# hyye/lio-mapping

Hardware: AMD Instinct MI355X
Metric: sliding-window solves/sec, 64-line 130k-pt scans, window=15 (opt_window=5) (higher is better)
Workload: dtype f64 (solve) / f32 (features); 1 GPU; HDL-64E outdoor_test_config_64, S_outdoor ray-cast scans, window_size=15 opt_window_size=5, one SolveOptimization per step, clouds resident in HBM; n_lidar_residuals=78236, local_map_points=76752, surf_stack_points=19386, parallelism=1 window

## Files before the change

### lio-mapping_amd/csrc/cloud_device.h

```cpp
#pragma once
#include <hip/hip_runtime.h>

#include <cfloat>
#include <climits>
#include <cstddef>

#include "cloud_kernels.h"
#include "hmath.h"
#include "knn_merge.h"

#if defined(__HIPCC__)
namespace lio {

__device__ inline bool finite3(const float4 &p) { return isfinite(p.x) && isfinite(p.y) && isfinite(p.z); }
__device__ inline bool finite3(const Vec3<float> &p) { return isfinite(p.x) && isfinite(p.y) && isfinite(p.z); }


template <bool NORMALISE_CONJ>
__device__ __forceinline__ float4 to_end_point(float4 p, float s, const Quat<float> &qe, const Vec3<float> &te) {
  p.x -= s * te.x; p.y -= s * te.y; p.z -= s * te.z;
  Quat<float> qid;
  Quat<float> qs = slerp(qid, s, qe, FLT_EPSILON);
  Quat<float> qc = conj(qs);
  if (NORMALISE_CONJ) qc = normalized(qc);
  Vec3<float> v = rotate(qc, Vec3<float>(p.x, p.y, p.z));
  v = rotate(qe, v);
  p.x = v.x + te.x; p.y = v.y + te.y; p.z = v.z + te.z;
  return p;
}
template <bool KEEP>
__device__ __forceinline__ float4 deskew_to_end_point(float4 p, const Quat<float> &qe, const Vec3<float> &te, float time_factor) {
  float s = time_factor * (p.w - int(p.w));
  if (!KEEP) p.w -= int(p.w);
  return to_end_point<true>(p, s, qe, te);
}
__device__ __forceinline__ float4 affine_map_point(const float *__restrict__ m, const float4 &p) {
  float4 o;
  o.x = m[0] * p.x + m[1] * p.y + m[2] * p.z + m[3];
  o.y = m[4] * p.x + m[5] * p.y + m[6] * p.z + m[7];
  o.z = m[8] * p.x + m[9] * p.y + m[10] * p.z + m[11];
  o.w = p.w;
  return o;
}
template <class B> __device__ __forceinline__ const float4 *concat_src(B *base, const float4 *p) { return rebase(base, p); }
__device__ __forceinline__ const float4 *concat_src(std::nullptr_t, const float4 *p) { return p; }
template <class B>
__device__ __forceinline__ float4 concat_point(const ConcatSeg *__restrict__ seg, int nseg, int g, B base) {
  int sidx = 0;
  for (int k = 1; k < nseg; ++k)
    if (g >= seg[k].dst_off) sidx = k;
  const ConcatSeg &sg = seg[sidx];
  const float4 p = concat_src(base, sg.src)[g - sg.dst_off];
  float4 o;
  if (sg.identity) o = p;
  else o = affine_map_point(sg.tf.m, p);
  if (sg.set_intensity) o.w = sg.intensity;
  return o;
}
__device__ __forceinline__ void odo_to_end_body(const float4 *in, float4 *out, const int i, const OdomState *__restrict__ st, float time_factor,
                                                int no_deskew) {
  Quat<float> qe(st->T[3], st->T[0], st->T[1], st->T[2]);
  Vec3<float> te(st->T[4], st->T[5], st->T[6]);
  float4 p = in[i];
  float s = time_factor * (p.w - int(p.w));
  if (no_deskew) s = 0;
  p.w = float(int(p.w));
  out[i] = to_end_point<false>(p, s, qe, te);
}
__device__ __forceinline__ float4 rigid_map_point(float4 p, const Quat<float> &q, const Vec3<float> &t) {
  const Vec3<float> v = rotate(q, Vec3<float>(p.x, p.y, p.z));
  return make_float4(v.x + t.x, v.y + t.y, v.z + t.z, p.w);
}

__device__ inline int cell_coord(float v, float inv_cell) { return int(floorf(v * inv_cell)); }
__device__ __forceinline__ bool cell_of(float x, float y, float z, const GridDesc &g, int &cx, int &cy, int &cz) {
  cx = cell_coord(x, g.inv_cell) - g.origin[0];
  cy = cell_coord(y, g.inv_cell) - g.origin[1];
  cz = cell_coord(z, g.inv_cell) - g.origin[2];
  return cx >= 0 && cy >= 0 && cz >= 0 && cx < g.dims[0] && cy < g.dims[1] && cz < g.dims[2];
}
__device__ __forceinline__ uint32_t cell_index(int cx, int cy, int cz, const GridDesc &g) { return uint32_t(cx + g.dims[0] * (cy + g.dims[1] * cz)); }
__device__ __forceinline__ uint32_t cell_key_clamped(const float4 &p, const GridDesc &g) {
  int cx, cy, cz;
  cell_of(p.x, p.y, p.z, g, cx, cy, cz);
  cx = min(max(cx, 0), g.dims[0] - 1); cy = min(max(cy, 0), g.dims[1] - 1); cz = min(max(cz, 0), g.dims[2] - 1);
  return cell_index(cx, cy, cz, g);
}

__device__ __forceinline__ void cell_count_point(const float4 *__restrict__ pts, int i, const GridDesc &g, uint32_t *__restrict__ keys,
                                                 uint32_t *__restrict__ slot, int *__restrict__ cnt) {
  const uint32_t c = cell_key_clamped(pts[i], g);
  keys[i] = c;
  slot[i] = uint32_t(atomicAdd(&cnt[c], 1));
}
__device__ __forceinline__ void cell_place_point(const float4 *__restrict__ pts, const uint32_t *__restrict__ keys, const uint32_t *__restrict__ slot, int i,
                                                 const int *__restrict__ starts, float4 *__restrict__ sorted, int *__restrict__ cnt) {
  float4 p = pts[i];
  p.w = __int_as_float(i);
  const uint32_t c = keys[i];
  sorted[starts[c] + int(slot[i])] = p;
  cnt[c] = 0;
}

#define SEG_SCAN_THREADS 1024
#define SEG_SCAN_ITEMS 4
__device__ __forceinline__ void block_exclusive_scan(const int *__restrict__ in, int *__restrict__ out, int n, int base) {
  __shared__ int wsum[SEG_SCAN_THREADS / 64];
  const int tid = threadIdx.x, lane = tid & 63, wv = tid >> 6;
  int carry = base;
  for (int c0 = 0; c0 < n; c0 += SEG_SCAN_THREADS * SEG_SCAN_ITEMS) {
    const int i0 = c0 + tid * SEG_SCAN_ITEMS;
    int v[SEG_SCAN_ITEMS], tsum = 0;
#pragma unroll
    for (int k = 0; k < SEG_SCAN_ITEMS; ++k) { v[k] = i0 + k < n ? in[i0 + k] : 0; tsum += v[k]; }
    int inc = tsum;
#pragma unroll
    for (int off = 1; off < 64; off <<= 1) {
      const int u = __shfl_up(inc, off, 64);
      if (lane >= off) inc += u;
    }
    if (lane == 63) wsum[wv] = inc;
    __syncthreads();
    int before = 0, total = 0;
#pragma unroll
    for (int w = 0; w < SEG_SCAN_THREADS / 64; ++w) { const int t = wsum[w]; if (w < wv) before += t; total += t; }
    int run = carry + before + inc - tsum;
#pragma unroll
    for (int k = 0; k < SEG_SCAN_ITEMS; ++k)
      if (i0 + k < n) { out[i0 + k] = run; run += v[k]; }
    carry += total;
    __syncthreads();
  }
}

#define VOX_TILE 256
#define VOX_KEY_NONE 0xFFFFFFFFu

template <int ZBITS>
__device__ __forceinline__ bool vox_abs_key(const float4 &p, float inv_leaf, uint32_t &key) {
  constexpr int ZOFF = 1 << (ZBITS - 1);
  const float cx = floorf(p.x * inv_leaf), cy = floorf(p.y * inv_leaf), cz = floorf(p.z * inv_leaf);
  if (!(fabsf(cx) < 1024.f && fabsf(cy) < 1024.f && fabsf(cz) < float(ZOFF - 1))) return false;
  key = (uint32_t(int(cz) + ZOFF) << 22) | (uint32_t(int(cy) + 1024) << 11) | uint32_t(int(cx) + 1024);
  return true;
}
template <int ZBITS, uint32_t NONE>
__device__ __forceinline__ uint32_t vox_take_point(const float4 &p, float inv_leaf, float (&mn)[3], float (&mx)[3], float &cnt, int *__restrict__ flag) {
  uint32_t key = NONE;
  if (finite3(p)) {
    cnt = 1.f;
    mn[0] = mx[0] = p.x; mn[1] = mx[1] = p.y; mn[2] = mx[2] = p.z;
    if (!vox_abs_key<ZBITS>(p, inv_leaf, key)) *flag = 1;
  }
  return key;
}

__device__ __forceinline__ void vox_block_partial(float (&mn)[3], float (&mx)[3], float cnt, float *__restrict__ row) {
  __shared__ float sm[7][VOX_TILE / 64];
  const int lane = threadIdx.x & 63, wv = threadIdx.x >> 6;
#pragma unroll
  for (int o = 32; o > 0; o >>= 1) {
    for (int d = 0; d < 3; ++d) { mn[d] = fminf(mn[d], __shfl_xor(mn[d], o, 64)); mx[d] = fmaxf(mx[d], __shfl_xor(mx[d], o, 64)); }
    cnt += __shfl_xor(cnt, o, 64);
  }
  if (lane == 0) { for (int d = 0; d < 3; ++d) { sm[d][wv] = mn[d]; sm[3 + d][wv] = mx[d]; } sm[6][wv] = cnt; }
  __syncthreads();
  if (threadIdx.x < 7) {
    const int t = threadIdx.x;
    float v = sm[t][0];
    for (int w = 1; w < VOX_TILE / 64; ++w) v = t < 3 ? fminf(v, sm[t][w]) : (t < 6 ? fmaxf(v, sm[t][w]) : v + sm[t][w]);
    row[t] = v;
  }
}
__device__ __forceinline__ void cloud_bounds_block(const float4 *__restrict__ pts, int n, int block, int nb, float *__restrict__ row) {
  float mn[3] = {FLT_MAX, FLT_MAX, FLT_MAX}, mx[3] = {-FLT_MAX, -FLT_MAX, -FLT_MAX};
  float cnt = 0;
  for (int i = block * VOX_TILE + threadIdx.x; i < n; i += nb * VOX_TILE) {
    const float4 p = pts[i];
    if (!finite3(p)) continue;
    cnt += 1.f;
    mn[0] = fminf(mn[0], p.x); mn[1] = fminf(mn[1], p.y); mn[2] = fminf(mn[2], p.z);
    mx[0] = fmaxf(mx[0], p.x); mx[1] = fmaxf(mx[1], p.y); mx[2] = fmaxf(mx[2], p.z);
  }
  vox_block_partial(mn, mx, cnt, row);
}

__device__ __forceinline__ bool vox_fold_bounds(const float *__restrict__ partial, int nb, float inv_leaf, VoxParams &v) {
  __shared__ float sm[7][VOX_TILE];
  const int t = threadIdx.x;
  float mn[3] = {FLT_MAX, FLT_MAX, FLT_MAX}, mx[3] = {-FLT_MAX, -FLT_MAX, -FLT_MAX};
  float cnt = 0;
  for (int b = t; b < nb; b += VOX_TILE) {
    for (int d = 0; d < 3; ++d) { mn[d] = fminf(mn[d], partial[size_t(b) * 8 + d]); mx[d] = fmaxf(mx[d], partial[size_t(b) * 8 + 3 + d]); }
    cnt += partial[size_t(b) * 8 + 6];
  }
  for (int d = 0; d < 3; ++d) { sm[d][t] = mn[d]; sm[3 + d][t] = mx[d]; }
  sm[6][t] = cnt;
  __syncthreads();
  for (int st = VOX_TILE / 2; st > 0; st >>= 1) {
    if (t < st) {
      for (int d = 0; d < 3; ++d) { sm[d][t] = fminf(sm[d][t], sm[d][t + st]); sm[3 + d][t] = fmaxf(sm[3 + d][t], sm[3 + d][t + st]); }
      sm[6][t] += sm[6][t + st];
    }
    __syncthreads();
  }
  if (t != 0) return false;
  long long dd[3];
  for (int d = 0; d < 3; ++d) {
    v.mn[d] = sm[d][0]; v.mx[d] = sm[3 + d][0];
    dd[d] = (long long)((v.mx[d] - v.mn[d]) * inv_leaf) + 1;
    v.minb[d] = int(floorf(v.mn[d] * inv_leaf));
    const int maxb = int(floorf(v.mx[d] * inv_leaf));
    v.divb[d] = maxb - v.minb[d] + 1;
  }
  v.overflow = (sm[6][0] > 0 && dd[0] * dd[1] * dd[2] > (long long)INT_MAX) ? 1 : 0;
  v.n_valid = int(sm[6][0]);
  return true;
}

__device__ __forceinline__ bool vox_is_head(const uint32_t *__restrict__ keys, int i, uint32_t k) {
  return k != VOX_KEY_NONE && (i == 0 || keys[i - 1] != k);
}
__device__ __forceinline__ void vox_tile_head_count(const uint32_t *__restrict__ keys, int n, int tile, int *__restrict__ count) {
  __shared__ int swave[VOX_TILE / 64];
  const int i = tile * VOX_TILE + threadIdx.x;
  const uint32_t k = i < n ? keys[i] : VOX_KEY_NONE;
  const unsigned long long b = __ballot(vox_is_head(keys, i, k));
  if ((threadIdx.x & 63) == 0) swave[threadIdx.x >> 6] = __popcll(b);
  __syncthreads();
  if (threadIdx.x == 0) *count = (swave[0] + swave[1]) + (swave[2] + swave[3]);
}

struct VoxSlot { int pos; bool head; };
__device__ __forceinline__ VoxSlot vox_centroid_tile(const float4 *__restrict__ pts, const uint32_t *__restrict__ keys, const uint32_t *__restrict__ vals,
                                                     const int *__restrict__ tile_heads, int n, int tile, float4 *__restrict__ out) {
  __shared__ float4 sp[VOX_TILE];
  __shared__ uint32_t sk[VOX_TILE];
  __shared__ int swave[VOX_TILE / 64], sbase[VOX_TILE / 64];
  const int tid = threadIdx.x, lane = tid & 63, wv = tid >> 6;
  const int base_i = tile * VOX_TILE, i = base_i + tid;
  int before = 0;
  for (int b = tid; b < tile; b += VOX_TILE) before += tile_heads[b];
#pragma unroll
  for (int o = 32; o > 0; o >>= 1) before += __shfl_xor(before, o, 64);
  const uint32_t k = i < n ? keys[i] : VOX_KEY_NONE;
  sk[tid] = k;
  if (k != VOX_KEY_NONE) sp[tid] = pts[vals[i]];
  const bool head = vox_is_head(keys, i, k);
  const unsigned long long hb = __ballot(head);
  if (lane == 0) { swave[wv] = __popcll(hb); sbase[wv] = before; }
  __syncthreads();
  int pos = (sbase[0] + sbase[1]) + (sbase[2] + sbase[3]);
  for (int w = 0; w < wv; ++w) pos += swave[w];
  pos += __popcll(hb & ((1ull << lane) - 1ull));
  if (head) {
    float ax = 0, ay = 0, az = 0, ai = 0;
    int e = tid;
    while (e < VOX_TILE && sk[e] == k) { const float4 p = sp[e]; ax += p.x; ay += p.y; az += p.z; ai += p.w; ++e; }
    int cnt = e - tid;
    if (e == VOX_TILE) {
      int g = base_i + VOX_TILE;
      while (g < n && keys[g] == k) { const float4 p = pts[vals[g]]; ax += p.x; ay += p.y; az += p.z; ai += p.w; ++g; ++cnt; }
    }
    const float c = float(cnt);
    out[pos] = make_float4(ax / c, ay / c, az / c, ai / c);
  }
  return VoxSlot{pos, head};
}

#define VSORT_THREADS 256
#define VSORT_SCATTER_THREADS 512
#define VSORT_SCATTER_ITEMS 2

__device__ __forceinline__ unsigned long long vsort_from_lane(unsigned long long v, int byte_addr) {
  const uint32_t lo = uint32_t(__builtin_amdgcn_ds_bpermute(byte_addr, int(uint32_t(v))));
  const uint32_t hi = uint32_t(__builtin_amdgcn_ds_bpermute(byte_addr, int(uint32_t(v >> 32))));
  return (static_cast<unsigned long long>(hi) << 32) | lo;
}

template <int E>
__device__ __forceinline__ void vsort_block(unsigned long long (&v)[E], unsigned long long *__restrict__ lds) {
  constexpr int P = VSORT_THREADS * E;
  const int base = int(threadIdx.x) * E, lane = int(threadIdx.x) & 63;
#pragma unroll 1
  for (int k = 2; k <= P; k <<= 1) {
// ... 599 lines not shown
```

### lio-mapping_amd/csrc/cloud_kernels.h

```cpp
#pragma once
#include <algorithm>
#include <cmath>
#include <cstdint>

#include "dev.h"
#include "hmath.h"

namespace lio {

struct VoxParams {
  float mn[3], mx[3];
  int minb[3], divb[3];
  int overflow;
  int n_valid;
};

struct Affine3f { float m[12]; };

#define LIO_MAX_FRAMES 32

struct ConcatSeg { const float4 *src; int n; int dst_off; int identity; int set_intensity; float intensity; Affine3f tf; };
struct ConcatArgs { ConcatSeg seg[LIO_MAX_FRAMES]; int nseg; int total; };
void launch_transform_concat(const ConcatArgs &a, float4 *dst, hipStream_t s);

void launch_deskew_to_end(float4 *pts, int n, const float q[4], const float p[3], float time_factor, hipStream_t s, bool keep_intensity = false);
void launch_rigid_map(const float4 *in, int n, const float q[4], const float p[3], float4 *out, hipStream_t s);

inline int cloud_bounds_blocks(int n) { return std::max(1, std::min(cdiv(n, 256), 512)); }
struct BoundsSeg { const float4 *pts; int n, nb, off; };
void launch_seg_bounds(const BoundsSeg *d_segs, int nseg, int max_nb, float *partial, float inv_leaf, VoxParams *d_out, hipStream_t s);

#define VSORT_CAP 4096
#define VSORT_MEAN 384
#define VSORT_OVERSAMPLE 8
#define VSORT_MAX_BUCKETS 1024
#define VSORT_MAX_N (VSORT_MAX_BUCKETS * VSORT_MEAN)
enum VoxSortPath { VSORT_PATH_SAMPLE = 0, VSORT_PATH_SINGLE = 1, VSORT_PATH_LIBRARY = 2 };
inline int vsort_buckets(size_t n) { return int((n + VSORT_MEAN - 1) / VSORT_MEAN); }

class VoxelGridDev {
 public:
  void sort_stats(unsigned long long out[3]) const { for (int k = 0; k < 3; ++k) out[k] = n_path_[k]; }
  int sort_pairs_hook(const uint32_t *keys, size_t n, uint32_t *keys_out, uint32_t *vals_out, hipStream_t s);
  size_t run(const float4 *in, size_t n, float leaf, DBuf<float4> &out, hipStream_t s, VoxParams *host_params = nullptr);
  void launch(const float4 *in, size_t n, float leaf, DBuf<float4> &out, hipStream_t s);
  size_t finish(VoxParams *host_params = nullptr);
  void set_host_signal(bool on) { use_signal_ = on; }
  VoxelGridDev() = default;
  VoxelGridDev(const VoxelGridDev &) = delete;
  VoxelGridDev &operator=(const VoxelGridDev &) = delete;

 private:
  const float4 *p_in_ = nullptr; size_t p_n_ = 0; DBuf<float4> *p_out_ = nullptr; hipStream_t p_stream_ = nullptr;
  float p_leaf_ = 0.f;
  void enqueue(bool exact, bool library);
  void reserve_sort(size_t n, hipStream_t s);
  int enqueue_sort(size_t n, hipStream_t s, bool library);
  DBuf<uint32_t> splitters_;
  DBuf<int> fill_;
  DBuf<unsigned long long> pairs_;
  int last_path_ = VSORT_PATH_LIBRARY;
  unsigned long long n_path_[3] = {0, 0, 0};
  HostBuf<char> h_mail_;
  int *h_count_ = nullptr;
  VoxParams *h_params_ = nullptr;
  DBuf<float> partial_;
  DBuf<VoxParams> params_;
  DBuf<uint32_t> keys_, keys2_, vals_, vals2_;
  DBuf<int> count_, tile_heads_;
  DBuf<char> tmp_;
  unsigned *h_flag_ = nullptr;
  unsigned seq_ = 0;
  HostSignal sig_{};
  bool use_signal_ = true;
};

struct GridDesc {
  int origin[3];
  int dims[3];
  float inv_cell;
  int n_points;
};

inline float knn_cell_edge(float min_match_sq_dis) { return std::sqrt(min_match_sq_dis) * 1.0001f + 1e-6f; }
inline float scan_to_map_cell_edge(float min_match_sq_dis) { return std::sqrt(min_match_sq_dis) * 1.0001f; }
inline void host_cloud_bounds(const float *xyzi, size_t n, float mn[3], float mx[3]) {
  for (int d = 0; d < 3; ++d) { mn[d] = 0.f; mx[d] = 0.f; }
  bool first = true;
  for (size_t i = 0; i < n; ++i) {
    const float *p = xyzi + 4 * i;
    if (!std::isfinite(p[0]) || !std::isfinite(p[1]) || !std::isfinite(p[2])) continue;
    for (int d = 0; d < 3; ++d) {
      if (first || p[d] < mn[d]) mn[d] = p[d];
      if (first || p[d] > mx[d]) mx[d] = p[d];
    }
    first = false;
  }
}
inline size_t grid_extent(GridDesc &g, const float mn[3], const float mx[3], float cell) {
  g.inv_cell = 1.0f / cell;
  size_t ncells = 1;
  for (int d = 0; d < 3; ++d) {
    const int lo = int(std::floor(mn[d] * g.inv_cell)) - 1, hi = int(std::floor(mx[d] * g.inv_cell)) + 1;
    g.origin[d] = lo; g.dims[d] = hi - lo + 1;
    ncells *= size_t(g.dims[d]);
  }
  return ncells;
}

class KnnGrid {
 public:
  void build(const float4 *pts, size_t n, const float mn[3], const float mx[3], float cell, hipStream_t s);
  const float4 *sorted() const { return sorted_.p; }
  const int *cells() const { return cells_.p; }
  const GridDesc &desc() const { return desc_; }

 private:
  GridDesc desc_{};
  DBuf<uint32_t> keys_, keys2_, vals_, vals2_;
  DBuf<float4> sorted_;
  DBuf<int> cells_, cnt_;
  bool cnt_dirty_ = false;
  DBuf<char> tmp_;
};

struct GridSeg { const float4 *pts; GridDesc g; int pt_off, cell_off, ncells; };
class GridBatch {
 public:
  void *begin(size_t head_bytes, int clouds);
  const void *head_dev() const { return d_tab_.p; }
  void add(const float4 *pts, int n);
  const VoxParams *bounds(hipStream_t s, float inv_leaf = 1.0f);
  void layout(float cell, size_t cells_cap);
  bool shared(int i) const { return gseg(i).pt_off >= 0; }
  const GridDesc &desc(int i) const { return gseg(i).g; }
  const float4 *sorted(int) const { return sorted_.p; }
  const int *cells(int i) const { return cells_.p + gseg(i).cell_off; }
  void build(hipStream_t s);

 private:
  BoundsSeg *bseg() { return reinterpret_cast<BoundsSeg *>(h_tab_.data() + off_b_); }
  GridSeg &gseg(int i) const { return reinterpret_cast<GridSeg *>(const_cast<char *>(h_tab_.data()) + off_g_)[i]; }
  std::vector<char> h_tab_;
  DBuf<char> d_tab_;
  size_t off_b_ = 0, off_g_ = 0, part_total_ = 0;
  int n_ = 0, max_nb_ = 0, max_pts_ = 0;
  bool any_shared_ = false;
  DBuf<float> partial_;
  DBuf<VoxParams> d_bounds_;
  HostBuf<VoxParams> h_bounds_;
  DBuf<uint32_t> keys_, slot_;
  DBuf<int> cnt_, cells_;
  DBuf<float4> sorted_;
  bool cnt_dirty_ = false;
};

struct FeatFrame { const float4 *stack; int M; int slot_off; int tf_index; const uint32_t *order = nullptr; };
struct FeatArgs {
  FeatFrame fr[LIO_MAX_FRAMES];
  int nframes;
  int max_M;
  float min_match_sq_dis, min_plane_dis;
  int mapping_mode;
  float fixed_pz[3];
};
void launch_features(const FeatArgs &a, const float *transforms, const float4 *map_sorted, const int *cells, const GridDesc &g,
                     uint8_t *valid, float4 *coef, float *score, const int *skip_flag, hipStream_t s);

void launch_knn(const float4 *query, int m, int k, float radius_sq, const float4 *map_sorted, const int *cells, const GridDesc &g,
                int32_t *idx, float *sqd, hipStream_t s);
void launch_knn_walk(const float4 *query, int m, int lanes_per_query, const float4 *map_sorted, const int *cells, const GridDesc &g,
                     int32_t *idx, float *sqd, float *nbr_xyz, hipStream_t s);

void launch_fit_five(int form, float min_match_sq_dis, float min_plane_dis, const float fixed_pz[3], const float *transform, const float4 *stack,
                     int m, const float4 *nbr, const float *fifth_sqd, uint8_t *valid, float4 *coef, float *score, float4 *abs_coef, hipStream_t s);

struct SolveSetup {
  float tf[LIO_MAX_FRAMES][8];
  int ntf;
  float odom_T[8];
  int set_odom;
};
struct OdomState;
void launch_solve_setup(const SolveSetup &a, float *d_transforms, OdomState *d_odom, uint8_t *valid, size_t n_valid, hipStream_t s);

struct OdomState {
  float T[8];
  int converged;
  int iters;
  int degenerate;
  int kz;
  int nsel;
};
inline OdomState odom_state_at(const Rigid<float> &T) {
  OdomState st{};
  st.T[0] = T.rot.x; st.T[1] = T.rot.y; st.T[2] = T.rot.z; st.T[3] = T.rot.w;
  st.T[4] = T.pos.x; st.T[5] = T.pos.y; st.T[6] = T.pos.z;
  return st;
}
inline void point_on_z_axis(const Rigid<float> &T, float pz[3]) {
  const Vec3<float> z = rotate(T.rot, Vec3<float>(0.f, 0.f, 10.f));
  pz[0] = z.x + T.pos.x; pz[1] = z.y + T.pos.y; pz[2] = z.z + T.pos.z;
}
class StateMail {
 public:
  void reserve(int n) {
    if (cap_ >= size_t(n)) return;
    cap_ = size_t(n) + size_t(n) / 2;
    buf_.alloc(cap_ * (STATE_MAIL_STRIDE + sizeof(unsigned)), hipHostMallocCoherent, true);
  }
  char *base() const { return buf_.p; }
  OdomState &slot(int j) const { return *reinterpret_cast<OdomState *>(buf_.p + size_t(j) * STATE_MAIL_STRIDE); }
  const HostSignal &arm(int n) {
    sig_.flag = reinterpret_cast<unsigned *>(buf_.p + cap_ * STATE_MAIL_STRIDE); sig_.seq = ++seq_; sig_.nslots = n;
    return sig_;
  }
  void wait(hipStream_t s) const { wait_host_signal(sig_, s); }
  bool all_converged(int n) const {
    bool all = true;
    for (int j = 0; j < n; ++j) all = all && slot(j).converged;
    return all;
  }

 private:
  HostBuf<char> buf_;
  size_t cap_ = 0;
  unsigned seq_ = 0;
  HostSignal sig_{};
};
static_assert(sizeof(OdomState) <= STATE_MAIL_STRIDE, "mailbox layout");

int odom_rows_blocks(int nslots);
int odom_round_blocks(int M, int lpq);
void launch_odom_round(const FeatArgs &a, int base_slot, int round, int keep, OdomState *st, const float4 *map_sorted, const int *cells, const GridDesc &g,
                       uint8_t *valid, float4 *coef, float *score, double *partials, hipStream_t s, OdomState *mail = nullptr,
                       const HostSignal &sig = HostSignal(), int lpq = 8);

void launch_gn_rows_map(const float4 *stack, int m, const uint8_t *valid, const float4 *coef, const OdomState *st, int b_from_coef, uint8_t *ok_out,
                        float *rows_out, hipStream_t s);
void launch_gn_fold(const double *partials, int nblocks, int wide, double *sums_out, hipStream_t s);
void launch_gn_step(const double *sums, OdomState *st, int iter, int min_rows, int left_update, hipStream_t s);

struct KfDesc {
  int slot_off, Mc, Ms;
  int map;
  int nb;
  int part_off;
  float pz[3];
};
struct KfMapDesc {
  const float4 *corner_sorted; const int *corner_cells; GridDesc corner_grid;
  const float4 *surf_sorted; const int *surf_cells; GridDesc surf_grid;
};
void launch_kf_query_keys(const KfDesc *kd, const KfMapDesc *md, const OdomState *st, int n_keyframes, int max_Mc, int max_Ms, const float4 *stack_all, uint32_t *keys,
                          hipStream_t s);
void launch_kf_round(const KfDesc *kd, const KfMapDesc *md, const OdomState *st, int n_keyframes, int max_Mc, int max_Ms, int lpq, const float4 *stack_all,
                     const uint32_t *order_or_null, float min_match_sq_dis, float min_plane_dis, int mapping_mode, uint8_t *valid, float4 *coef,
                     float4 *abs_coef_or_null, hipStream_t s);
void launch_kf_rows(const KfDesc *kd, const OdomState *st, int n_keyframes, int max_nb, const float4 *stack_all, const uint8_t *valid, const float4 *coef,
                    double *partials, int b_from_coef, hipStream_t s);
void launch_kf_update(const KfDesc *kd, OdomState *st, int n_keyframes, const double *partials, int iter, int min_rows, int left_update, int *n_converged,
                      char *mail, const HostSignal &sig, hipStream_t s);

#if defined(__HIPCC__)
__device__ inline void reduce_partials28(const double *__restrict__ partials, int nblocks, double *ssum ) {
  __shared__ double part28[8][32];
  const int c = threadIdx.x & 31, g = threadIdx.x >> 5;
  double v = 0;
  if (c < 28 && g < 8)
    for (int b = g; b < nblocks; b += 8) v += partials[b * 28 + c];
  if (g < 8) part28[g][c] = v;
  __syncthreads();
  if (threadIdx.x < 28) {
    double s = 0;
#pragma unroll
    for (int k = 0; k < 8; ++k) s += part28[k][threadIdx.x];
// ... 8 lines not shown
```

### lio-mapping_amd/csrc/cloud_kernels.hip

```cpp
#include <cstring>
#include <hip/hip_runtime.h>
#include <rocprim/rocprim.hpp>

#include <cfloat>
#include <climits>

#include "cloud_kernels.h"
#include "cloud_device.h"

namespace lio {

__global__ void k_transform_concat(ConcatArgs a, float4 *__restrict__ dst) {
  int gid = blockIdx.x * blockDim.x + threadIdx.x;
  if (gid >= a.total) return;
  dst[gid] = concat_point(a.seg, a.nseg, gid, nullptr);
}

void launch_transform_concat(const ConcatArgs &a, float4 *dst, hipStream_t s) {
  if (a.total <= 0) return;
  hipLaunchKernelGGL(k_transform_concat, dim3(cdiv(a.total, 256)), dim3(256), 0, s, a, dst);
  LIO_HIP(hipGetLastError());
}

template <bool KEEP>
// ... 195 lines not shown
      __syncthreads();
      if (tid < 64) post_host_mail(sig, mail, &smail, int(sizeof(VoxMail) / 4), tid);
    }
  }
}

void VoxelGridDev::launch(const float4 *in, size_t n, float leaf, DBuf<float4> &out, hipStream_t s) {
  p_in_ = in; p_n_ = n; p_out_ = &out; p_stream_ = s; p_leaf_ = leaf;
  if (n == 0) return;
  enqueue(false, false);
}

void VoxelGridDev::enqueue(bool exact, bool library) {
  const float4 *in = p_in_;
  const size_t n = p_n_;
  DBuf<float4> &out = *p_out_;
  hipStream_t s = p_stream_;
  const int ni = int(n);
  const float inv_leaf = 1.0f / p_leaf_;
  const int nkb = cdiv(ni, VOX_TILE);
  partial_.reserve(size_t(std::max(nkb, 512)) * 8);
  params_.reserve(1);
  reserve_sort(n, s);
  out.reserve(n);
  if (!h_count_) {
    h_mail_.alloc(256, hipHostMallocCoherent, true);
    static_assert(sizeof(VoxMail) <= 128, "mailbox layout");
    h_count_ = reinterpret_cast<int *>(h_mail_.p);
    h_params_ = reinterpret_cast<VoxParams *>(h_count_ + 1);
    h_flag_ = reinterpret_cast<unsigned *>(reinterpret_cast<char *>(h_count_) + 128);
  }
  int *d_range = count_.p + 1;
  if (!use_signal_) LIO_HIP(hipMemsetAsync(d_range, 0, sizeof(int), s));
  int npartial = 0;
  if (exact) {
    const int nb = cloud_bounds_blocks(ni);
    hipLaunchKernelGGL(k_cloud_bounds, dim3(nb), dim3(VOX_TILE), 0, s, in, ni, partial_.p);
    hipLaunchKernelGGL(k_cloud_bounds_fold, dim3(1), dim3(VOX_TILE), 0, s, partial_.p, nb, inv_leaf, params_.p);
    hipLaunchKernelGGL(k_vox_keys, dim3(cdiv(ni, 256)), dim3(256), 0, s, in, ni, inv_leaf, params_.p, keys_.p, vals_.p);
  } else {
    hipLaunchKernelGGL(k_vox_keys_abs, dim3(nkb), dim3(VOX_TILE), 0, s, in, ni, inv_leaf, keys_.p, vals_.p, partial_.p, d_range);
    npartial = nkb;
  }
  last_path_ = enqueue_sort(n, s, library);
  const int ntiles = cdiv(ni, VOX_TILE);
  tile_heads_.reserve(ntiles);
  hipLaunchKernelGGL(k_vox_tile_heads, dim3(ntiles + 1), dim3(VOX_TILE), 0, s, keys2_.p, ni, tile_heads_.p, partial_.p, npartial, inv_leaf, params_.p);
  sig_ = HostSignal();
  if (use_signal_) { sig_.flag = h_flag_; sig_.seq = ++seq_; }

  hipLaunchKernelGGL(k_vox_centroids, dim3(ntiles), dim3(VOX_TILE), 0, s, in, keys2_.p, vals2_.p, tile_heads_.p, ni, out.p, count_.p, params_.p, d_range,
                     count_.p + 2, reinterpret_cast<VoxMail *>(h_count_), sig_);
  LIO_HIP(hipGetLastError());
  if (!sig_.flag) {
    VoxMail *m = reinterpret_cast<VoxMail *>(h_count_);
    LIO_HIP(hipMemcpyAsync(&m->count, count_.p, sizeof(int), hipMemcpyDeviceToHost, s));
    LIO_HIP(hipMemcpyAsync(&m->params, params_.p, sizeof(VoxParams), hipMemcpyDeviceToHost, s));
    LIO_HIP(hipMemcpyAsync(&m->range_overflow, d_range, sizeof(int), hipMemcpyDeviceToHost, s));
    LIO_HIP(hipMemcpyAsync(&m->sort_overflow, count_.p + 2, sizeof(int), hipMemcpyDeviceToHost, s));
  }
}

void VoxelGridDev::reserve_sort(size_t n, hipStream_t s) {
  keys_.reserve(n); keys2_.reserve(n); vals_.reserve(n); vals2_.reserve(n);
  if (count_.cap < 3) { count_.reserve(3); LIO_HIP(hipMemsetAsync(count_.p, 0, count_.cap * sizeof(int), s)); }
}

int VoxelGridDev::enqueue_sort(size_t n, hipStream_t s, bool library) {
  const int ni = int(n);
  int *d_overflow = count_.p + 2;
  if (library || n > size_t(VSORT_MAX_N)) {
    LIO_HIP(hipMemsetAsync(d_overflow, 0, sizeof(int), s));
    size_t tmp_bytes = 0;
    LIO_HIP(rocprim::radix_sort_pairs(nullptr, tmp_bytes, keys_.p, keys2_.p, vals_.p, vals2_.p, n, 0, 32, s));
    tmp_.reserve(tmp_bytes + 256);
    LIO_HIP(rocprim::radix_sort_pairs(tmp_.p, tmp_bytes, keys_.p, keys2_.p, vals_.p, vals2_.p, n, 0, 32, s));
    return VSORT_PATH_LIBRARY;
  }
  if (ni <= VSORT_CAP) {
    hipLaunchKernelGGL(k_vsort_single, dim3(cdiv(ni, VSORT_THREADS / VSORT_RANK_LANES)), dim3(VSORT_THREADS), 0, s, keys_.p, ni, d_overflow, keys2_.p, vals2_.p);
    return VSORT_PATH_SINGLE;
  }
  const int NB = vsort_buckets(n);
  splitters_.reserve(NB); fill_.reserve(NB); pairs_.reserve(size_t(NB) * VSORT_CAP);
  hipLaunchKernelGGL(k_vsort_splitters, dim3(cdiv(VSORT_OVERSAMPLE * NB, VSORT_THREADS / VSORT_RANK_LANES)), dim3(VSORT_THREADS), 0, s, keys_.p, ni, NB,
                     splitters_.p, fill_.p, d_overflow);
  hipLaunchKernelGGL(k_vsort_scatter, dim3(cdiv(ni, VSORT_SCATTER_THREADS * VSORT_SCATTER_ITEMS)), dim3(VSORT_SCATTER_THREADS), 0, s, keys_.p, ni, NB,
                     splitters_.p, fill_.p, pairs_.p, d_overflow);
  hipLaunchKernelGGL(k_vsort_buckets, dim3(NB), dim3(VSORT_THREADS), 0, s, pairs_.p, fill_.p, NB, ni, d_overflow, keys2_.p, vals2_.p);
  return VSORT_PATH_SAMPLE;
}

int VoxelGridDev::sort_pairs_hook(const uint32_t *keys, size_t n, uint32_t *keys_out, uint32_t *vals_out, hipStream_t s) {
  reserve_sort(n, s);
  std::vector<uint32_t> iota(n);
  for (size_t i = 0; i < n; ++i) iota[i] = uint32_t(i);
  LIO_HIP(hipMemcpyAsync(keys_.p, keys, n * sizeof(uint32_t), hipMemcpyHostToDevice, s));
  LIO_HIP(hipMemcpyAsync(vals_.p, iota.data(), n * sizeof(uint32_t), hipMemcpyHostToDevice, s));
  int path = enqueue_sort(n, s, false);
  LIO_HIP(hipGetLastError());
  int overflow = 0;
  LIO_HIP(hipMemcpyAsync(&overflow, count_.p + 2, sizeof(int), hipMemcpyDeviceToHost, s));
  LIO_HIP(hipStreamSynchronize(s));
  if (overflow) path = enqueue_sort(n, s, true);
  LIO_HIP(hipMemcpyAsync(keys_out, keys2_.p, n * sizeof(uint32_t), hipMemcpyDeviceToHost, s));
  LIO_HIP(hipMemcpyAsync(vals_out, vals2_.p, n * sizeof(uint32_t), hipMemcpyDeviceToHost, s));
  LIO_HIP(hipStreamSynchronize(s));
  return path;
}

size_t VoxelGridDev::finish(VoxParams *host_params) {
  if (p_n_ == 0) {
    if (host_params) std::memset(host_params, 0, sizeof(*host_params));
    return 0;
  }
  const VoxMail *m = reinterpret_cast<const VoxMail *>(h_count_);
  bool redone = false, exact = false, library = false;
  for (;;) {
    if (sig_.flag) wait_host_signal(sig_, p_stream_);
    else LIO_HIP(hipStreamSynchronize(p_stream_));
    if (m->range_overflow == 1 && !exact) {
      exact = true;
      enqueue(exact, library);
      redone = true;
      continue;
    }
    if (m->sort_overflow == 1 && !library) {
      library = true;
      enqueue(exact, library);
      redone = true;
      continue;
    }
    if (redone) LIO_HIP(hipStreamSynchronize(p_stream_));
    break;
  }
  ++n_path_[last_path_];
  int count = m->count;
  const VoxParams hp = m->params;
  if (hp.overflow) {
    p_out_->reserve(p_n_);
    LIO_HIP(hipMemcpyAsync(p_out_->p, p_in_, p_n_ * sizeof(float4), hipMemcpyDeviceToDevice, p_stream_));
    LIO_HIP(hipStreamSynchronize(p_stream_));
    count = int(p_n_);
  }
  if (host_params) *host_params = hp;
  return size_t(count);
}

size_t VoxelGridDev::run(const float4 *in, size_t n, float leaf, DBuf<float4> &out, hipStream_t s, VoxParams *host_params) {
  launch(in, n, leaf, out, s);
  return finish(host_params);
}

__global__ void k_cell_count(const float4 *__restrict__ pts, int n, GridDesc g, uint32_t *__restrict__ keys, uint32_t *__restrict__ slot,
                             int *__restrict__ cnt) {
  int i = blockIdx.x * blockDim.x + threadIdx.x;
  if (i >= n) return;
  cell_count_point(pts, i, g, keys, slot, cnt);
}

__global__ void k_cell_place(const float4 *__restrict__ pts, const uint32_t *__restrict__ keys, const uint32_t *__restrict__ slot, int n,
                             const int *__restrict__ starts, float4 *__restrict__ sorted, int *__restrict__ cnt) {
  int i = blockIdx.x * blockDim.x + threadIdx.x;
  if (i >= n) return;
  cell_place_point(pts, keys, slot, i, starts, sorted, cnt);
}

void KnnGrid::build(const float4 *pts, size_t n, const float mn[3], const float mx[3], float cell, hipStream_t s) {
  desc_.n_points = int(n);
  const size_t ncells = grid_extent(desc_, mn, mx, cell);
  if (ncells > (size_t(1) << 30)) throw DeviceError("KnnGrid: cell table too large");
  cells_.reserve(ncells + 1);
  if (cnt_.cap < ncells + 1 || cnt_dirty_) {
    cnt_.reserve(ncells + 1);
    LIO_HIP(hipMemsetAsync(cnt_.p, 0, cnt_.cap * sizeof(int), s));
  }
  cnt_dirty_ = true;
  keys_.reserve(std::max<size_t>(n, 1)); vals_.reserve(std::max<size_t>(n, 1)); sorted_.reserve(std::max<size_t>(n, 1));
  const int ni = int(n);
  if (ni) hipLaunchKernelGGL(k_cell_count, dim3(cdiv(ni, 256)), dim3(256), 0, s, pts, ni, desc_, keys_.p, vals_.p, cnt_.p);
  size_t tmp_bytes = 0;
  LIO_HIP(rocprim::exclusive_scan(nullptr, tmp_bytes, cnt_.p, cells_.p, 0, ncells + 1, rocprim::plus<int>(), s));
  tmp_.reserve(tmp_bytes + 256);
  LIO_HIP(rocprim::exclusive_scan(tmp_.p, tmp_bytes, cnt_.p, cells_.p, 0, ncells + 1, rocprim::plus<int>(), s));
  if (ni) hipLaunchKernelGGL(k_cell_place, dim3(cdiv(ni, 256)), dim3(256), 0, s, pts, keys_.p, vals_.p, ni, cells_.p, sorted_.p, cnt_.p);
  LIO_HIP(hipGetLastError());
  cnt_dirty_ = false;
}

__global__ void __launch_bounds__(256) k_seg_cell_count(const GridSeg *__restrict__ segs, uint32_t *__restrict__ keys, uint32_t *__restrict__ slot,
                                                        int *__restrict__ cnt) {
  const GridSeg &r = segs[blockIdx.y];
  const int i = blockIdx.x * blockDim.x + threadIdx.x;
  if (r.pt_off < 0 || i >= r.g.n_points) return;
  cell_count_point(r.pts, i, r.g, keys + r.pt_off, slot + r.pt_off, cnt + r.cell_off);
}
__global__ void __launch_bounds__(SEG_SCAN_THREADS) k_seg_cell_scan(const GridSeg *__restrict__ segs, const int *__restrict__ cnt, int *__restrict__ cells) {
  const GridSeg &r = segs[blockIdx.x];
  if (r.pt_off < 0) return;
  block_exclusive_scan(cnt + r.cell_off, cells + r.cell_off, r.ncells + 1, r.pt_off);
}
__global__ void __launch_bounds__(256) k_seg_cell_place(const GridSeg *__restrict__ segs, const uint32_t *__restrict__ keys, const uint32_t *__restrict__ slot,
                                                        const int *__restrict__ cells, float4 *__restrict__ sorted, int *__restrict__ cnt) {
  const GridSeg &r = segs[blockIdx.y];
  const int i = blockIdx.x * blockDim.x + threadIdx.x;
  if (r.pt_off < 0 || i >= r.g.n_points) return;
  cell_place_point(r.pts, keys + r.pt_off, slot + r.pt_off, i, cells + r.cell_off, sorted, cnt + r.cell_off);
}

void *GridBatch::begin(size_t head_bytes, int clouds) {
  off_g_ = head_bytes; off_b_ = off_g_ + size_t(clouds) * sizeof(GridSeg);
  h_tab_.assign(off_b_ + size_t(clouds) * sizeof(BoundsSeg), 0);
  d_tab_.reserve(std::max<size_t>(h_tab_.size(), 1));
  n_ = max_nb_ = max_pts_ = 0; part_total_ = 0;
  any_shared_ = false;
  return h_tab_.data();
}
void GridBatch::add(const float4 *pts, int n) {
  const int nb = cloud_bounds_blocks(n);
  bseg()[n_++] = BoundsSeg{pts, n, nb, int(part_total_)};
  part_total_ += size_t(nb);
  max_nb_ = std::max(max_nb_, nb); max_pts_ = std::max(max_pts_, n);
}
const VoxParams *GridBatch::bounds(hipStream_t s, float inv_leaf) {
  partial_.reserve(part_total_ * 8); d_bounds_.reserve(size_t(n_));
  if (h_bounds_.n < size_t(n_)) h_bounds_.alloc(size_t(n_) + size_t(n_) / 2, hipHostMallocDefault);
  LIO_HIP(hipMemcpyAsync(d_tab_.p + off_b_, h_tab_.data() + off_b_, size_t(n_) * sizeof(BoundsSeg), hipMemcpyHostToDevice, s));
  launch_seg_bounds(reinterpret_cast<const BoundsSeg *>(d_tab_.p + off_b_), n_, max_nb_, partial_.p, inv_leaf, d_bounds_.p, s);
  LIO_HIP(hipMemcpyAsync(h_bounds_.p, d_bounds_.p, size_t(n_) * sizeof(VoxParams), hipMemcpyDeviceToHost, s));
  LIO_HIP(hipStreamSynchronize(s));
  return h_bounds_.p;
}
void GridBatch::layout(float cell, size_t cells_cap) {
  size_t cell_total = 0, pt_off = 0;
  for (int i = 0; i < n_; ++i) {
    VoxParams &b = h_bounds_.p[i];
    if (b.n_valid == 0)
      for (int e = 0; e < 3; ++e) b.mn[e] = b.mx[e] = 0.f;
    GridSeg &g = gseg(i);
    g.pts = bseg()[i].pts; g.g.n_points = bseg()[i].n; g.pt_off = -1;
    const size_t ncells = grid_extent(g.g, b.mn, b.mx, cell);
    if (ncells > cells_cap) continue;
    g.pt_off = int(pt_off); g.cell_off = int(cell_total); g.ncells = int(ncells);
    pt_off += size_t(g.g.n_points); cell_total += ncells + 1;
    if (pt_off > size_t(INT_MAX) || cell_total > size_t(INT_MAX)) throw CapacityError("GridBatch: the points or the cell tables exceed 2^31 entries");
    any_shared_ = true;
  }
  cells_.reserve(std::max<size_t>(cell_total, 1));
  if (cnt_.cap < std::max<size_t>(cell_total, 1)) { cnt_.reserve(std::max<size_t>(cell_total, 1)); cnt_dirty_ = true; }
  keys_.reserve(std::max<size_t>(pt_off, 1)); slot_.reserve(std::max<size_t>(pt_off, 1)); sorted_.reserve(std::max<size_t>(pt_off, 1));
}
void GridBatch::build(hipStream_t s) {
  if (any_shared_ && cnt_dirty_) LIO_HIP(hipMemsetAsync(cnt_.p, 0, cnt_.cap * sizeof(int), s));
  LIO_HIP(hipMemcpyAsync(d_tab_.p, h_tab_.data(), off_b_, hipMemcpyHostToDevice, s));
  if (!any_shared_) return;
  const GridSeg *segs = reinterpret_cast<const GridSeg *>(d_tab_.p + off_g_);
  const int pb = cdiv(max_pts_, 256);
  cnt_dirty_ = true;
  if (pb) hipLaunchKernelGGL(k_seg_cell_count, dim3(pb, n_), dim3(256), 0, s, segs, keys_.p, slot_.p, cnt_.p);
  hipLaunchKernelGGL(k_seg_cell_scan, dim3(n_), dim3(SEG_SCAN_THREADS), 0, s, segs, cnt_.p, cells_.p);
  if (pb) hipLaunchKernelGGL(k_seg_cell_place, dim3(pb, n_), dim3(256), 0, s, segs, keys_.p, slot_.p, cells_.p, sorted_.p, cnt_.p);
  LIO_HIP(hipGetLastError());
  cnt_dirty_ = false;
}

#define KNN_WALK_THREADS 256
template <int K, int LPQ>
__global__ void __launch_bounds__(KNN_WALK_THREADS) k_nn_walk(const float4 *__restrict__ query, int m, int cut, float radius_sq,
                                                              const float4 *__restrict__ map, const int *__restrict__ cells, GridDesc g,
                                                              int32_t *__restrict__ idx, float *__restrict__ sqd, float *__restrict__ nbr) {
  const int gt = blockIdx.x * blockDim.x + threadIdx.x;
  const int i = gt / LPQ, sub = gt % LPQ;
  const bool active = i < m;
  const float4 q4 = active ? query[i] : make_float4(0, 0, 0, 0);
  float bd[K]; int bi[K], bj[K];
  knn_scan_group<K, LPQ>(Vec3<float>(q4.x, q4.y, q4.z), active, sub, map, cells, g, bd, bi, bj);
  if (!active || sub != 0) return;
#pragma unroll
  for (int k = 0; k < K; ++k) {
    const bool ok = bi[k] != INT_MAX && !(cut && !(bd[k] < radius_sq));
    const size_t o = size_t(i) * K + k;
    idx[o] = ok ? bi[k] : -1;
    sqd[o] = ok ? bd[k] : INFINITY;
    if (nbr) {
      const float4 p = ok ? map[bj[k]] : make_float4(0, 0, 0, 0);
      nbr[3 * o + 0] = p.x; nbr[3 * o + 1] = p.y; nbr[3 * o + 2] = p.z;
    }
  }
}

template <int K, int LPQ>
static void launch_knn_walk_as(const float4 *query, int m, int cut, float radius_sq, const float4 *map_sorted, const int *cells, const GridDesc &g,
                               int32_t *idx, float *sqd, float *nbr, hipStream_t s) {
  hipLaunchKernelGGL((k_nn_walk<K, LPQ>), dim3(cdiv((long long)m * LPQ, KNN_WALK_THREADS)), dim3(KNN_WALK_THREADS), 0, s, query, m, cut, radius_sq,
                     map_sorted, cells, g, idx, sqd, nbr);
}

void launch_knn(const float4 *query, int m, int k, float radius_sq, const float4 *map_sorted, const int *cells, const GridDesc &g,
                int32_t *idx, float *sqd, hipStream_t s) {
  if (m <= 0) return;
  if (k == 1) launch_knn_walk_as<1, 8>(query, m, 1, radius_sq, map_sorted, cells, g, idx, sqd, nullptr, s);
  else if (k == 5) launch_knn_walk_as<5, 8>(query, m, 1, radius_sq, map_sorted, cells, g, idx, sqd, nullptr, s);
  else throw DeviceError("launch_knn: k is 1 or 5");
  LIO_HIP(hipGetLastError());
}

void launch_knn_walk(const float4 *query, int m, int lanes_per_query, const float4 *map_sorted, const int *cells, const GridDesc &g,
                     int32_t *idx, float *sqd, float *nbr_xyz, hipStream_t s) {
  if (m <= 0) return;
  if (lanes_per_query == 1) launch_knn_walk_as<5, 1>(query, m, 0, 0.f, map_sorted, cells, g, idx, sqd, nbr_xyz, s);
  else if (lanes_per_query == 4) launch_knn_walk_as<5, 4>(query, m, 0, 0.f, map_sorted, cells, g, idx, sqd, nbr_xyz, s);
  else if (lanes_per_query == 8) launch_knn_walk_as<5, 8>(query, m, 0, 0.f, map_sorted, cells, g, idx, sqd, nbr_xyz, s);
  else throw DeviceError("launch_knn_walk: lanes per query is 1, 4 or 8");
  LIO_HIP(hipGetLastError());
}

template <bool MAPPING, int LPQ>
__global__ void __launch_bounds__(FEAT_THREADS) k_features(FeatArgs a, const float *__restrict__ transforms, const float4 *__restrict__ map,
                                                          const int *__restrict__ cells, GridDesc g, uint8_t *__restrict__ valid,
                                                          float4 *__restrict__ coef, float *__restrict__ score, const int *__restrict__ skip_flag,
                                                          float4 *__restrict__ abs_coef) {
  if (skip_flag && *skip_flag) return;
  features_block<MAPPING, LPQ>(a.fr[blockIdx.y], feat_scalars(a), int(blockIdx.x), transforms, map, cells, g, valid, coef, score, abs_coef);
}

__device__ __forceinline__ uint8_t line_features_fit(const Vec3<float> &t, const Vec3<float> &pz, const Vec3<float> &sel, float min_match_sq_dis,
                                                     float bd4, int bi4, const int (&bj)[5], const float4 *__restrict__ map, float4 &c) {
  uint8_t ok = 0;
  c = make_float4(0, 0, 0, 0);
  if (bi4 != INT_MAX && bd4 < min_match_sq_dis) {
    float nx[5], ny[5], nz[5];
    Vec3<float> vc(0.f, 0.f, 0.f);
#pragma unroll
    for (int j = 0; j < 5; ++j) {
      float4 pn = map[bj[j]];
      nx[j] = pn.x; ny[j] = pn.y; nz[j] = pn.z;
      vc.x += pn.x; vc.y += pn.y; vc.z += pn.z;
    }
// ... 351 lines not shown
```

Measured before the change: 2503 solves/s.

## Replace rocprim cell scan with tile-count single-pass scan in KnnGrid build

The count kernel now also accumulates per-tile point counts into sharded tile counters, using a wavefront ballot to merge runs that share a tile. A new single-pass scan kernel computes each tile's base from those counters, scans only tiles that hold points, and fills empty tiles with a constant. This replaces rocprim's multi-kernel exclusive scan and its temp buffer. The place kernel resets the tile counters so the zeroing memset can be skipped on later builds, at the cost of extra atomics and some added complexity.

```diff
diff --git a/lio-mapping_amd/csrc/cloud_device.h b/lio-mapping_amd/csrc/cloud_device.h
--- a/lio-mapping_amd/csrc/cloud_device.h
+++ b/lio-mapping_amd/csrc/cloud_device.h
@@ -87,32 +87,57 @@
   return cell_index(cx, cy, cz, g);
 }
 
+#define GRID_SCAN_TILE 4096
+#define GRID_SCAN_TILES_MAX 2048
+#define GRID_TILE_NONE 0xFFFFFFFFu
+#define GRID_TILE_SHARDS 16
+__device__ __forceinline__ int grid_tile_shard(unsigned block) { return int(block & (GRID_TILE_SHARDS - 1)); }
 __device__ __forceinline__ void cell_count_point(const float4 *__restrict__ pts, int i, const GridDesc &g, uint32_t *__restrict__ keys,
-                                                 uint32_t *__restrict__ slot, int *__restrict__ cnt) {
-  const uint32_t c = cell_key_clamped(pts[i], g);
-  keys[i] = c;
-  slot[i] = uint32_t(atomicAdd(&cnt[c], 1));
+                                                 uint32_t *__restrict__ slot, int *__restrict__ cnt, int *__restrict__ tile_cnt = nullptr,
+                                                 int tile_shift = 0, bool live = true) {
+  uint32_t tile = GRID_TILE_NONE;
+  if (live) {
+    const uint32_t c = cell_key_clamped(pts[i], g);
+    keys[i] = c;
+    slot[i] = uint32_t(atomicAdd(&cnt[c], 1));
+    tile = c >> tile_shift;
+  }
+  if (tile_cnt == nullptr) return;
+  const int lane = threadIdx.x & 63;
+  const uint32_t prev = __shfl_up(tile, 1, 64);
+  const bool head = lane == 0 || tile != prev;
+  const unsigned long long heads = __ballot(head);
+  if (head && tile != GRID_TILE_NONE) {
+    const unsigned long long later = lane == 63 ? 0ull : heads >> (lane + 1);
+    atomicAdd(tile_cnt + tile, later ? __ffsll(later) : 64 - lane);
+  }
 }
 __device__ __forceinline__ void cell_place_point(const float4 *__restrict__ pts, const uint32_t *__restrict__ keys, const uint32_t *__restrict__ slot, int i,
-                                                 const int *__restrict__ starts, float4 *__restrict__ sorted, int *__restrict__ cnt) {
+                                                 const int *__restrict__ starts, float4 *__restrict__ sorted, int *__restrict__ cnt,
+                                                 int *__restrict__ tile_cnt = nullptr, int tile_shift = 0) {
   float4 p = pts[i];
   p.w = __int_as_float(i);
   const uint32_t c = keys[i];
   sorted[starts[c] + int(slot[i])] = p;
   cnt[c] = 0;
+  if (tile_cnt) tile_cnt[c >> tile_shift] = 0;
 }
 
 #define SEG_SCAN_THREADS 1024
 #define SEG_SCAN_ITEMS 4
-__device__ __forceinline__ void block_exclusive_scan(const int *__restrict__ in, int *__restrict__ out, int n, int base) {
+template <class BaseFn>
+__device__ __forceinline__ void block_exclusive_scan_from(const int *__restrict__ in, int *__restrict__ out, int n, BaseFn base_fn) {
   __shared__ int wsum[SEG_SCAN_THREADS / 64];
   const int tid = threadIdx.x, lane = tid & 63, wv = tid >> 6;
-  int carry = base;
+  int carry = 0;
   for (int c0 = 0; c0 < n; c0 += SEG_SCAN_THREADS * SEG_SCAN_ITEMS) {
     const int i0 = c0 + tid * SEG_SCAN_ITEMS;
     int v[SEG_SCAN_ITEMS], tsum = 0;
 #pragma unroll
-    for (int k = 0; k < SEG_SCAN_ITEMS; ++k) { v[k] = i0 + k < n ? in[i0 + k] : 0; tsum += v[k]; }
+    for (int k = 0; k < SEG_SCAN_ITEMS; ++k) v[k] = i0 + k < n ? in[i0 + k] : 0;
+    if (c0 == 0) carry = base_fn();
+#pragma unroll
+    for (int k = 0; k < SEG_SCAN_ITEMS; ++k) tsum += v[k];
     int inc = tsum;
 #pragma unroll
     for (int off = 1; off < 64; off <<= 1) {
@@ -131,6 +156,9 @@
     carry += total;
     __syncthreads();
   }
+}
+__device__ __forceinline__ void block_exclusive_scan(const int *__restrict__ in, int *__restrict__ out, int n, int base) {
+  block_exclusive_scan_from(in, out, n, [base] { return base; });
 }
 
 #define VOX_TILE 256
diff --git a/lio-mapping_amd/csrc/cloud_kernels.h b/lio-mapping_amd/csrc/cloud_kernels.h
--- a/lio-mapping_amd/csrc/cloud_kernels.h
+++ b/lio-mapping_amd/csrc/cloud_kernels.h
@@ -119,9 +119,8 @@
   GridDesc desc_{};
   DBuf<uint32_t> keys_, keys2_, vals_, vals2_;
   DBuf<float4> sorted_;
-  DBuf<int> cells_, cnt_;
+  DBuf<int> cells_, cnt_, tile_cnt_;
   bool cnt_dirty_ = false;
-  DBuf<char> tmp_;
 };
 
 struct GridSeg { const float4 *pts; GridDesc g; int pt_off, cell_off, ncells; };
diff --git a/lio-mapping_amd/csrc/cloud_kernels.hip b/lio-mapping_amd/csrc/cloud_kernels.hip
--- a/lio-mapping_amd/csrc/cloud_kernels.hip
+++ b/lio-mapping_amd/csrc/cloud_kernels.hip
@@ -371,18 +371,53 @@
   return finish(host_params);
 }
 
-__global__ void k_cell_count(const float4 *__restrict__ pts, int n, GridDesc g, uint32_t *__restrict__ keys, uint32_t *__restrict__ slot,
-                             int *__restrict__ cnt) {
+__global__ void __launch_bounds__(256) k_cell_count(const float4 *__restrict__ pts, int n, GridDesc g, uint32_t *__restrict__ keys,
+                                                    uint32_t *__restrict__ slot, int *__restrict__ cnt, int *__restrict__ tile_cnt, int tile_shift) {
+  const int i = blockIdx.x * blockDim.x + threadIdx.x;
+  cell_count_point(pts, i, g, keys, slot, cnt, tile_cnt + grid_tile_shard(blockIdx.x) * GRID_SCAN_TILES_MAX, tile_shift, i < n);
+}
+
+static_assert(GRID_TILE_SHARDS == SEG_SCAN_THREADS / 64, "k_cell_scan_tiles: one wavefront per shard");
+static_assert(GRID_SCAN_TILE == SEG_SCAN_THREADS * SEG_SCAN_ITEMS && GRID_SCAN_TILES_MAX % 4 == 0, "k_cell_scan_tiles: tile and chunk");
+__global__ void __launch_bounds__(SEG_SCAN_THREADS) k_cell_scan_tiles(const int *__restrict__ cnt, const int *__restrict__ tile_cnt,
+                                                                      int *__restrict__ cells, int n, int tile_shift) {
+  __shared__ int part[SEG_SCAN_THREADS / 64];
+  const int b = blockIdx.x, tid = threadIdx.x, lane = tid & 63, wv = tid >> 6;
+  int own = 0;
+#pragma unroll
+  for (int sh = 0; sh < GRID_TILE_SHARDS; ++sh) own += tile_cnt[sh * GRID_SCAN_TILES_MAX + b];
+  int sum = 0;
+  const int4 *row = reinterpret_cast<const int4 *>(tile_cnt + wv * GRID_SCAN_TILES_MAX);
+  for (int q = lane; 4 * q < b; q += 64) {
+    const int4 v = row[q];
+    sum += v.x + (4 * q + 1 < b ? v.y : 0) + (4 * q + 2 < b ? v.z : 0) + (4 * q + 3 < b ? v.w : 0);
+  }
+  auto base_of = [&] {
+#pragma unroll
+    for (int off = 32; off; off >>= 1) sum += __shfl_xor(sum, off, 64);
+    if (lane == 0) part[wv] = sum;
+    __syncthreads();
+    int base = 0;
+#pragma unroll
+    for (int w = 0; w < SEG_SCAN_THREADS / 64; ++w) base += part[w];
+    return base;
+  };
+  const long long off = (long long)b << tile_shift;
+  const int len = int(min(1ll << tile_shift, (long long)n - off));
+  if (own == 0) {
+    const int base = base_of();
+    for (int j = tid; j < len; j += SEG_SCAN_THREADS) cells[off + j] = base;
+    return;
+  }
+  block_exclusive_scan_from(cnt + off, cells + off, len, base_of);
+}
+
+__global__ void k_cell_place(const float4 *__restrict__ pts, const uint32_t *__restrict__ keys, const uint32_t *__restrict__ slot, int n,
+                             const int *__restrict__ starts, float4 *__restrict__ sorted, int *__restrict__ cnt, int *__restrict__ tile_cnt,
+                             int tile_shift) {
   int i = blockIdx.x * blockDim.x + threadIdx.x;
   if (i >= n) return;
-  cell_count_point(pts, i, g, keys, slot, cnt);
-}
-
-__global__ void k_cell_place(const float4 *__restrict__ pts, const uint32_t *__restrict__ keys, const uint32_t *__restrict__ slot, int n,
-                             const int *__restrict__ starts, float4 *__restrict__ sorted, int *__restrict__ cnt) {
-  int i = blockIdx.x * blockDim.x + threadIdx.x;
-  if (i >= n) return;
-  cell_place_point(pts, keys, slot, i, starts, sorted, cnt);
+  cell_place_point(pts, keys, slot, i, starts, sorted, cnt, tile_cnt + grid_tile_shard(blockIdx.x) * GRID_SCAN_TILES_MAX, tile_shift);
 }
 
 void KnnGrid::build(const float4 *pts, size_t n, const float mn[3], const float mx[3], float cell, hipStream_t s) {
@@ -390,19 +425,22 @@
   const size_t ncells = grid_extent(desc_, mn, mx, cell);
   if (ncells > (size_t(1) << 30)) throw DeviceError("KnnGrid: cell table too large");
   cells_.reserve(ncells + 1);
-  if (cnt_.cap < ncells + 1 || cnt_dirty_) {
-    cnt_.reserve(ncells + 1);
+  int tile_shift = 0;
+  while ((1 << tile_shift) < GRID_SCAN_TILE) ++tile_shift;
+  while (((ncells + 1 + (size_t(1) << tile_shift) - 1) >> tile_shift) > GRID_SCAN_TILES_MAX) ++tile_shift;
+  const int tiles = int((ncells + 1 + (size_t(1) << tile_shift) - 1) >> tile_shift);
+  if (cnt_.cap < ncells + 1 || tile_cnt_.cap < size_t(GRID_TILE_SHARDS) * GRID_SCAN_TILES_MAX || cnt_dirty_) {
+    cnt_.reserve(ncells + 1); tile_cnt_.reserve(size_t(GRID_TILE_SHARDS) * GRID_SCAN_TILES_MAX);
     LIO_HIP(hipMemsetAsync(cnt_.p, 0, cnt_.cap * sizeof(int), s));
+    LIO_HIP(hipMemsetAsync(tile_cnt_.p, 0, tile_cnt_.cap * sizeof(int), s));
   }
   cnt_dirty_ = true;
   keys_.reserve(std::max<size_t>(n, 1)); vals_.reserve(std::max<size_t>(n, 1)); sorted_.reserve(std::max<size_t>(n, 1));
   const int ni = int(n);
-  if (ni) hipLaunchKernelGGL(k_cell_count, dim3(cdiv(ni, 256)), dim3(256), 0, s, pts, ni, desc_, keys_.p, vals_.p, cnt_.p);
-  size_t tmp_bytes = 0;
-  LIO_HIP(rocprim::exclusive_scan(nullptr, tmp_bytes, cnt_.p, cells_.p, 0, ncells + 1, rocprim::plus<int>(), s));
-  tmp_.reserve(tmp_bytes + 256);
-  LIO_HIP(rocprim::exclusive_scan(tmp_.p, tmp_bytes, cnt_.p, cells_.p, 0, ncells + 1, rocprim::plus<int>(), s));
-  if (ni) hipLaunchKernelGGL(k_cell_place, dim3(cdiv(ni, 256)), dim3(256), 0, s, pts, keys_.p, vals_.p, ni, cells_.p, sorted_.p, cnt_.p);
+  if (ni) hipLaunchKernelGGL(k_cell_count, dim3(cdiv(ni, 256)), dim3(256), 0, s, pts, ni, desc_, keys_.p, vals_.p, cnt_.p, tile_cnt_.p, tile_shift);
+  hipLaunchKernelGGL(k_cell_scan_tiles, dim3(tiles), dim3(SEG_SCAN_THREADS), 0, s, cnt_.p, tile_cnt_.p, cells_.p, int(ncells + 1), tile_shift);
+  if (ni)
+    hipLaunchKernelGGL(k_cell_place, dim3(cdiv(ni, 256)), dim3(256), 0, s, pts, keys_.p, vals_.p, ni, cells_.p, sorted_.p, cnt_.p, tile_cnt_.p, tile_shift);
   LIO_HIP(hipGetLastError());
   cnt_dirty_ = false;
 }
```

Result: no change. 2507 solves/s, median of 2 (+0.2%).
